# facebookresearch/brainmagick

Measured on AMD Instinct MI355X. Metric: segments/s, 208-ch x 360-sample SimpleConv + ClipLoss training step, higher is better.
Workload: dtype f32 (fp32-accurate: operands split into 2 scaled f16 planes, 3 MFMA products, fp32 accumulate; same parity tolerances as exact fp32, see DESIGN.md §2); 1 GPU; cfg2: gwilliams2022-shaped MEG C=208 T=360, F=120 features, 27 subjects, clip_conv SimpleConv (8985590 params) + ClipLoss + Adam; batch_per_gpu=256, global_batch=256, negatives=local, parallelism=dp1, comm=none, rccl_world=1, candidate_gather=none, distinct_batches=8

## Files before the change

### brainmagick_amd/csrc/bm_block.h

```cpp
#pragma once
#include "bm_common.h"

template <int V> struct BmVec;
template <> struct BmVec<1> {
    typedef float F;
    typedef unsigned char M;
};
template <> struct BmVec<4> {
    typedef f32x4 F;
    typedef uchar4 M;
};
__device__ __forceinline__ float bm_get(const float& v, int) { return v; }
__device__ __forceinline__ float bm_get(const f32x4& v, int i) { return v[i]; }
__device__ __forceinline__ unsigned char bm_get(const unsigned char& v, int) { return v; }
__device__ __forceinline__ unsigned char bm_get(const uchar4& v, int i) {
    return i == 0 ? v.x : i == 1 ? v.y : i == 2 ? v.z : v.w;
}
__device__ __forceinline__ void bm_set(float& v, int, float x) { v = x; }
__device__ __forceinline__ void bm_set(f32x4& v, int i, float x) { v[i] = x; }

template <int N, typename T, typename Op>
__device__ __forceinline__ T bm_pairwise(const T* v, Op op) {
    if constexpr (N == 1) return v[0];
    else return op(bm_pairwise<N / 2>(v, op), bm_pairwise<N - N / 2>(v + N / 2, op));
}
template <int WAVES, typename T, typename Op>
__device__ __forceinline__ T bm_block_fold(T wv, T* sh, Op op) {
    bm_wave_to_lds(wv, sh);
    __syncthreads();
    wv = bm_pairwise<WAVES>(sh, op);
    __syncthreads();
    return wv;
}
__device__ __forceinline__ float bm_max2(float a, float b) { return fmaxf(a, b); }
template <int WAVES>
__device__ __forceinline__ float bm_block_max(float v, float* sh) {
    return bm_block_fold<WAVES>(bm_wave_max(v), sh, bm_max2);
}
template <int WAVES>
__device__ __forceinline__ float bm_block_sum(float v, float* sh) {
    return bm_block_fold<WAVES>(bm_wave_sum(v), sh, [](float a, float b) { return a + b; });
}
template <int WAVES>
__device__ __forceinline__ double bm_block_sum(double v, double* sh) {
    return bm_block_fold<WAVES>(bm_wave_sum_d(v), sh, [](double a, double b) { return a + b; });
}

template <typename P>
struct BmFoldWs {
    unsigned* tickets;
    P* part;
    static constexpr long bytes(long n_partials) { return 64 + n_partials * (long)sizeof(P); }
    static BmFoldWs at(void* base) {
        return base ? BmFoldWs{(unsigned*)base, (P*)((char*)base + 64)} : BmFoldWs{nullptr, nullptr};
    }
};
template <typename T, int WAVES, int N = 1>
struct BmFoldLds {
    T wave[N][WAVES];
    int last;
};

template <typename P>
__device__ __forceinline__ void bm_store_partial(P* dst, P v) {
    __hip_atomic_store(dst, v, __ATOMIC_RELAXED, __HIP_MEMORY_SCOPE_AGENT);
}
__device__ __forceinline__ bool bm_last_arriver(unsigned* ticket, unsigned nblocks, int* sh_flag) {
    if (threadIdx.x == 0) {
        asm volatile("s_waitcnt vmcnt(0)" ::: "memory");
        const unsigned prev = __hip_atomic_fetch_add(ticket, 1u, __ATOMIC_RELAXED, __HIP_MEMORY_SCOPE_AGENT);
        const bool last = prev == nblocks - 1;
        if (last) {
            __builtin_amdgcn_fence(__ATOMIC_ACQUIRE, "agent");
            asm volatile("s_waitcnt vmcnt(0)" ::: "memory");
            __hip_atomic_store(ticket, 0u, __ATOMIC_RELAXED, __HIP_MEMORY_SCOPE_AGENT);
        }
        *sh_flag = last;
    }
    __syncthreads();
    return *sh_flag != 0;
}

template <int WAVES>
__device__ __forceinline__ bool bm_amax_arrive(float mx, float* part_dst, unsigned* ticket, unsigned nblocks,
                                               BmFoldLds<float, WAVES>& sh) {
    bm_wave_to_lds(bm_wave_max(mx), sh.wave[0]);
    __syncthreads();
    if (threadIdx.x == 0) bm_store_partial(part_dst, bm_pairwise<WAVES>(sh.wave[0], bm_max2));
    return bm_last_arriver(ticket, nblocks, &sh.last);
}
template <int WAVES>
__device__ __forceinline__ void bm_amax_slot_store(float m, float* out, float* sh) {
    bm_wave_to_lds(bm_wave_max(m), sh);
    __syncthreads();
    if (threadIdx.x < BM_AMAX_SHARDS) {
        float v = 0.f;
        if (threadIdx.x == 0) v = bm_pairwise<WAVES>(sh, bm_max2);
        out[threadIdx.x] = v;
    }
}
template <int WAVES>
__device__ __forceinline__ void bm_amax_fold(const float* part, int n, float* out, float* sh) {
    float m = 0.f;
    for (int i = threadIdx.x; i < n; i += WAVES * 64) m = fmaxf(m, part[i]);
    bm_amax_slot_store<WAVES>(m, out, sh);
}
template <int WAVES>
__device__ __forceinline__ void bm_amax_fold_rows(const float* part, int rows, int nsplit, int row_stride,
                                                  int split_stride, float* out, float* rows_out, float* sh) {
    float m = 0.f;
    for (int r = threadIdx.x; r < rows; r += WAVES * 64) {
        float v = 0.f;
        for (int k = 0; k < nsplit; ++k) v = fmaxf(v, part[r * row_stride + k * split_stride]);
        if (rows_out) rows_out[r] = v;
        m = fmaxf(m, v);
    }
    bm_amax_slot_store<WAVES>(m, out, sh);
}
```

### brainmagick_amd/csrc/conv_nn_h2w.hip

```cpp
#include "conv_h2_common.h"

#ifdef HG_TRACE
__device__ unsigned ch_trace_buf[64 * 4 * 24];
extern "C" int bm_debug_trace_read_conv(unsigned* out) {
    return (int)hipMemcpyFromSymbol(out, HIP_SYMBOL(ch_trace_buf), sizeof(unsigned) * 64 * 4 * 24);
}
#endif

__device__ __forceinline__ void ch_split_hi(float x0, float x1, float s, unsigned& hi) {
    asm("v_fma_mixlo_f16 %0, %1, %3, 0\n\t"
        "v_fma_mixhi_f16 %0, %2, %3, 0" : "=&v"(hi) : "v"(x0), "v"(x1), "v"(s));
}
__device__ __forceinline__ void ch_split_lo(float x0, float x1, float s, unsigned hi, unsigned& lo) {
    asm("v_fma_mixlo_f16 %0, %2, %4, -%1 op_sel_hi:[0,0,1]\n\t"
        "v_fma_mixhi_f16 %0, %3, %4, -%1 op_sel:[0,0,1] op_sel_hi:[0,0,1]"
        : "=&v"(lo) : "v"(hi), "v"(x0), "v"(x1), "v"(s));
}

enum { H2R_NONE = 0, H2R_WLOAD, H2R_SPLIT, H2R_WRITE, H2R_BAR, H2R_BREAD };
struct H2RItem { int kind, arg; };
template <int KS, int J, int NB>
constexpr int h2r_nitems() {
    if (KS == 1) return 32 + 4 + 1 + NB;
    return J == 0 ? 16 + NB : J == 1 ? 16 + 4 + 1 + NB : NB;
// ... 84 lines not shown
#define H2R_SOFF(C16_, J_) (((((C16_) >> 1) * KS + (J_)) * 8 + ((C16_) & 1) * 2) * a.Mpad * 16)
#define H2R_LOAD_X(R_, CB_) xreg[R_] = __builtin_bit_cast(float, __builtin_amdgcn_raw_buffer_load_b32(xr, (CB_) + (R_) * crow, 0, 0));
    const u32x4* xrd = Xs + h * HXWP + wn * (NW * 32) + nl;
    u32x4* xwr = Xs + tid;

    bm_static_for<16>([&](auto rc) __attribute__((always_inline)) { H2R_LOAD_X(decltype(rc)::value, xoff0) });
    bm_static_for<NA>([&](auto kc) __attribute__((always_inline)) { H2R_LOAD_A(0, decltype(kc)::value, 0) });
    bm_static_for<8>([&](auto uc) __attribute__((always_inline)) {
        constexpr int u = decltype(uc)::value;
        ch_split_hi(xreg[2 * u], xreg[2 * u + 1], sx, ph[u]);
        ch_split_lo(xreg[2 * u], xreg[2 * u + 1], sx, ph[u], pw[u]);
    });
    xwr[(0 * 2 + 0) * HXWP] = u32x4{ph[0], ph[1], ph[2], ph[3]};
    xwr[(1 * 2 + 0) * HXWP] = u32x4{pw[0], pw[1], pw[2], pw[3]};
    xwr[(0 * 2 + 1) * HXWP] = u32x4{ph[4], ph[5], ph[6], ph[7]};
    xwr[(1 * 2 + 1) * HXWP] = u32x4{pw[4], pw[5], pw[6], pw[7]};
    if (KS == 1) bm_static_for<16>([&](auto rc) __attribute__((always_inline)) { H2R_LOAD_X(decltype(rc)::value, 16 * crow + xoff0) });
    asm volatile("s_waitcnt lgkmcnt(0)\n\ts_barrier" ::: "memory");
    bm_static_for<NB>([&](auto ic) __attribute__((always_inline)) {
        constexpr int i = decltype(ic)::value;
        bf[0][i / NW][i % NW] = __builtin_bit_cast(f16x8, xrd[(i / NW) * 2 * HXWP + (i % NW) * 32]);
    });

#ifdef HG_TRACE
    unsigned tr[8], tacc[3][8];
    for (int i = 0; i < 3; ++i) for (int k = 0; k < 8; ++k) tacc[i][k] = 0;
    __builtin_amdgcn_sched_barrier(0);
    const unsigned t_loop0 = (unsigned)__builtin_readcyclecounter();
#endif
    auto stage = [&](int c16, auto jc, auto pc) __attribute__((always_inline)) {
        constexpr int j = decltype(jc)::value, par = decltype(pc)::value;
        CH_T(0)
        const bool last_chunk = c16 + 1 >= n16;
        const int nc16 = (j == KS - 1 && !last_chunk) ? c16 + 1 : c16;
        const int soff = (j == KS - 1) ? H2R_SOFF(nc16, last_chunk ? KS - 1 : 0) : H2R_SOFF(c16, j + 1);
        const u32x4* xnext = xrd + ((j == KS - 1 ? c16 + 1 : c16) & 1) * HXSLAB + (j == KS - 1 ? 0 : (j + 1) * a.dil);
        const int cb = (c16 + (KS == 1 ? 2 : 1)) * 16 * crow + xoff0;
        u32x4* xw = xwr + ((c16 + 1) & 1) * HXSLAB;
        bm_static_for<NS>([&](auto nc) __attribute__((always_inline)) {
            constexpr int n = decltype(nc)::value;
            constexpr int term = n / TN, w = n % TN, mt = w / NW, nt = w % NW;
            constexpr int pa = term == 0 ? 1 : 0, pb = term == 1 ? 1 : 0;
            acc[mt][nt] = __builtin_amdgcn_mfma_f32_32x32x16_f16(af[par][pa][mt], bf[par][pb][nt], acc[mt][nt], 0, 0, 0);
            if constexpr (n % 4 == 0) {
                if constexpr (n / 4 < NA) H2R_LOAD_A(par ^ 1, n / 4, soff)
            } else {
                constexpr int f = (n / 4) * 3 + n % 4 - 1;
                constexpr int L = h2r_nitems<KS, j, NB>();
                constexpr int i0 = (f * L + NF - 1) / NF, i1 = ((f + 1) * L + NF - 1) / NF;
                bm_static_for<i1 - i0>([&](auto ic) __attribute__((always_inline)) {
                    constexpr H2RItem it = h2r_item<KS, j, NB>(i0 + decltype(ic)::value);
                    if constexpr (it.kind == H2R_WLOAD) {
                        H2R_LOAD_X(it.arg, cb)
                    } else if constexpr (it.kind == H2R_SPLIT) {
                        constexpr int u = it.arg / 2;
                        if constexpr (it.arg % 2 == 0) ch_split_hi(xreg[2 * u], xreg[2 * u + 1], sx, ph[u]);
                        else ch_split_lo(xreg[2 * u], xreg[2 * u + 1], sx, ph[u], pw[u]);
                    } else if constexpr (it.kind == H2R_WRITE) {
                        constexpr int kg = it.arg / 2, plane = it.arg % 2;
                        if constexpr (plane == 0) xw[(0 * 2 + kg) * HXWP] = u32x4{ph[4 * kg], ph[4 * kg + 1], ph[4 * kg + 2], ph[4 * kg + 3]};
                        else xw[(1 * 2 + kg) * HXWP] = u32x4{pw[4 * kg], pw[4 * kg + 1], pw[4 * kg + 2], pw[4 * kg + 3]};
                    } else if constexpr (it.kind == H2R_BAR) {
                        asm volatile("s_waitcnt lgkmcnt(0)\n\ts_barrier" ::: "memory");
                    } else if constexpr (it.kind == H2R_BREAD) {
                        constexpr int p = it.arg / NW, q = it.arg % NW;
                        bf[par ^ 1][p][q] = __builtin_bit_cast(f16x8, xnext[p * 2 * HXWP + q * 32]);
                    }
                });
            }
            __builtin_amdgcn_sched_barrier(0);
        });
        CH_T(4)
#ifdef HG_TRACE
        tacc[j][0] += tr[4] - tr[0]; tacc[j][7] += 1;
#endif
    };
    auto chunk = [&](int c16, auto cpc) __attribute__((always_inline)) {
        constexpr int cp = decltype(cpc)::value;
        bm_static_for<KS>([&](auto jc) __attribute__((always_inline)) {
            constexpr int j = decltype(jc)::value;
            stage(c16, jc, std::integral_constant<int, (cp + j) & 1>{});
        });
    };
    for (int c16 = 0; c16 < n16; c16 += 2) {
        chunk(c16, std::integral_constant<int, 0>{});
        chunk(c16 + 1, std::integral_constant<int, KS & 1>{});
    }
#ifdef HG_TRACE
    __builtin_amdgcn_sched_barrier(0);
    const unsigned t_loop1 = (unsigned)__builtin_readcyclecounter();
    if (blockIdx.x < 64 && lane == 0)
        for (int i = 0; i < 3; ++i) for (int k = 0; k < 8; ++k) ch_trace_buf[((blockIdx.x * 4 + wave) * 3 + i) * 8 + k] = tacc[i][k];
#endif
    asm volatile("s_waitcnt vmcnt(0) lgkmcnt(0)\n\ts_barrier" ::: "memory");
#undef H2R_LOAD_A
#undef H2R_SOFF
#undef H2R_LOAD_X

#ifdef HG_TRACE
    h2_tile_epilogue<MW, RESK>(args, acc, smem, b, g, m0, n0, ntile, sx_inv, tid, lane, wm, wn, nl, h, ch_trace_buf);
#else
    h2_tile_epilogue<MW, RESK>(args, acc, smem, b, g, m0, n0, ntile, sx_inv, tid, lane, wm, wn, nl, h);
#endif
#ifdef HG_TRACE
    asm volatile("s_waitcnt vmcnt(0)" ::: "memory");
    if (blockIdx.x < 64 && lane == 0) {
        unsigned* o = ch_trace_buf + ((blockIdx.x * 4 + wave) * 3) * 8;
        o[5] = t_loop0 - t_kernel0;
        o[6] = (unsigned)__builtin_readcyclecounter() - t_loop1;
        o[8 + 5] = t_loop1 - t_loop0;
    }
#endif
}

extern "C" int bm_conv_h2_mw_for(int M) {
    int best = 5;
    long best_pad = -1;
    const int cand[3] = {5, 4, 2};
    for (int i = 0; i < 3; ++i) {
        const long bm = 64L * cand[i];
        const long pad = (long)cdiv(M, bm) * bm;
        if (best_pad < 0 || pad < best_pad) { best_pad = pad; best = cand[i]; }
    }
    return best;
}
extern "C" int bm_conv_h2_mpad(int M) {
    const int bm = 64 * bm_conv_h2_mw_for(M);
    return cdiv(M, bm) * bm;
}

extern "C" int bm_conv_h2_covers(int Cin, int M, int T, int KS, int dil) {
    if (KS != 1 && KS != 3) return 0;
    if ((KS >> 1) * dil > 16 || T <= 128) return 0;
    if ((long)Cin * T * 4 >= 0x40000000L) return 0;
    if ((long)Cin * KS > 3840) return 0;
    return (long)bm_conv_h2_mpad(M) * 2 <= (long)M * 3 || M >= 96;
}

extern "C" int bm_conv_h2_stats_tiles(int B, int T) { return B * cdiv(T, HBN) * 2; }

extern "C" long bm_packed_weight_bytes_h2(int G, int M, int Cin, int KS) {
    const long mpad = bm_conv_h2_mpad(M);
    return (long)G * cdiv(Cin, 32) * KS * 2 * 4 * mpad * 8 * 2 + (long)G * mpad * 4;
}

struct PackH2Job {
    const float* src;
    unsigned short* dst;
    float* wscale;
    const float* alpha;
    long sg, sm, sc, sj;
    int M, Cin, KS, flip, Mpad, nchunk;
    int block0, nblocks;
};

#define PACK_ROWS 4
#define PACK_MAX_NK 3840

__device__ __forceinline__ void pack_h2_rows(const PackH2Job& jb, int block, float* tile, float* rs) {
    const float* __restrict__ src = jb.src;
    const int M = jb.M, Cin = jb.Cin, KS = jb.KS, Mpad = jb.Mpad, nchunk = jb.nchunk, flip = jb.flip;
    const long sg = jb.sg, sm = jb.sm, sc = jb.sc, sj = jb.sj;
    const int rows_per_group = Mpad / PACK_ROWS;
    const int g = block / rows_per_group, m0 = (block - g * rows_per_group) * PACK_ROWS;
    const float alpha = jb.alpha ? *jb.alpha : 1.f;
    const int nk = Cin * KS;
    const int tid = threadIdx.x, lane = tid & 63, wave = tid >> 6;
    const float* base = src + g * sg + (long)m0 * sm;
    const bool rows_inside = sm < sc;
    for (int idx = tid; idx < PACK_ROWS * nk; idx += blockDim.x) {
        int r, c, j;
        if (rows_inside) {
            j = idx % KS;
            const int t = idx / KS;
            r = t % PACK_ROWS;
            c = t / PACK_ROWS;
        } else {
            j = idx % KS;
            const int t = idx / KS;
            c = t % Cin;
            r = t / Cin;
        }
        tile[r * nk + c * KS + j] = (m0 + r < M) ? alpha * base[r * sm + c * sc + j * sj] : 0.f;
    }
    __syncthreads();
    {
        float mx = 0.f;
        for (int i = lane; i < nk; i += 64) mx = fmaxf(mx, fabsf(tile[wave * nk + i]));
        mx = bm_wave_max(mx);
        float s, inv;
        bm_scale_from_amax(mx, s, inv);
        if (lane == 0) {
            rs[wave] = s;
            jb.wscale[(long)g * Mpad + m0 + wave] = inv;
        }
    }
    __syncthreads();
    const int nslots = nchunk * KS * 4;
    const long plane_stride = (long)4 * Mpad * 8;
    for (int t = tid; t < PACK_ROWS * nslots; t += blockDim.x) {
        const int r = t % PACK_ROWS, q = t / PACK_ROWS;
        const int kg = q & 3;
        const int j = (q >> 2) % KS;
        const int chunk = (q >> 2) / KS;
        const int jj = flip ? KS - 1 - j : j;
        const float sr = rs[r];
        alignas(16) unsigned short hi[8];
        alignas(16) unsigned short lo[8];
#pragma unroll
        for (int e8 = 0; e8 < 8; ++e8) {
            const int c = chunk * 32 + kg * 8 + e8;
            const float v = c < Cin ? tile[r * nk + c * KS + jj] * sr : 0.f;
            const _Float16 a = (_Float16)v;
            const _Float16 l = (_Float16)(v - (float)a);
            hi[e8] = __builtin_bit_cast(unsigned short, a);
            lo[e8] = __builtin_bit_cast(unsigned short, l);
        }
        const long stage = ((long)g * nchunk + chunk) * KS + j;
        unsigned short* out = jb.dst + stage * 2 * plane_stride + ((long)kg * Mpad + m0 + r) * 8;
        *reinterpret_cast<uint4*>(out) = *reinterpret_cast<const uint4*>(hi);
        *reinterpret_cast<uint4*>(out + plane_stride) = *reinterpret_cast<const uint4*>(lo);
    }
}

__global__ __launch_bounds__(256) void pack_weights_h2_kernel(PackH2Job jb) {
    extern __shared__ float pack_smem[];
    pack_h2_rows(jb, blockIdx.x, pack_smem + PACK_ROWS, pack_smem);
}

__global__ __launch_bounds__(256) void pack_weights_h2_batch_kernel(const PackH2Job* __restrict__ jobs, int njobs) {
    extern __shared__ float pack_smem[];
    int lo = 0, hi = njobs - 1;
    while (lo < hi) {
        const int mid = (lo + hi + 1) >> 1;
        if (jobs[mid].block0 <= (int)blockIdx.x) lo = mid; else hi = mid - 1;
    }
    const PackH2Job jb = jobs[lo];
    pack_h2_rows(jb, blockIdx.x - jb.block0, pack_smem + PACK_ROWS, pack_smem);
}

static int pack_h2_fill(PackH2Job& jb, const float* src, void* dst, int G, int M, int Cin, int KS, long sg, long sm,
                        long sc, long sj, int flip, const float* alpha_ptr) {
    BM_REQUIRE(src && dst, "pack_weights_h2: null pointer");
    BM_REQUIRE(G > 0 && M > 0 && Cin > 0 && KS > 0, "pack_weights_h2: bad dims");
    jb.Mpad = bm_conv_h2_mpad(M);
    jb.nchunk = cdiv(Cin, 32);
    const long f16_elems = (long)G * jb.nchunk * KS * 2 * 4 * jb.Mpad * 8;
    jb.src = src; jb.dst = (unsigned short*)dst;
    jb.wscale = reinterpret_cast<float*>(reinterpret_cast<char*>(dst) + f16_elems * 2);
    jb.alpha = alpha_ptr;
    jb.sg = sg; jb.sm = sm; jb.sc = sc; jb.sj = sj;
    jb.M = M; jb.Cin = Cin; jb.KS = KS; jb.flip = flip;
    BM_REQUIRE(Cin * KS <= PACK_MAX_NK, "pack_weights_h2: Cin * KS = %d exceeds %d", Cin * KS, PACK_MAX_NK);
    jb.block0 = 0; jb.nblocks = G * jb.Mpad / PACK_ROWS;
    return BM_OK;
}

extern "C" int bm_pack_weights_h2(const float* src, void* dst, int G, int M, int Cin, int KS, long sg, long sm,
                                  long sc, long sj, int flip, const float* alpha_ptr, void* stream) {
    PackH2Job jb;
    if (int rc = pack_h2_fill(jb, src, dst, G, M, Cin, KS, sg, sm, sc, sj, flip, alpha_ptr)) return rc;
    hipLaunchKernelGGL(pack_weights_h2_kernel, dim3((unsigned)jb.nblocks), dim3(256),
                       (size_t)(PACK_ROWS + PACK_ROWS * Cin * KS) * sizeof(float), (hipStream_t)stream, jb);
    return bm_check_launch("pack_weights_h2");
}

extern "C" int bm_pack_h2_job_bytes() { return (int)sizeof(PackH2Job); }

extern "C" int bm_pack_h2_job_fill(void* job, const float* src, void* dst, int G, int M, int Cin, int KS, long sg,
                                   long sm, long sc, long sj, int flip, const float* alpha_ptr, int block0) {
    if (!job) return -1;
    PackH2Job jb;
    if (pack_h2_fill(jb, src, dst, G, M, Cin, KS, sg, sm, sc, sj, flip, alpha_ptr)) return -1;
    jb.block0 = block0;
    memcpy(job, &jb, sizeof(jb));
    return jb.nblocks;
}

extern "C" int bm_pack_weights_h2_batch(const void* jobs_dev, int njobs, int total_blocks, int max_nk, void* stream) {
    BM_REQUIRE(jobs_dev && njobs > 0 && total_blocks > 0, "pack_weights_h2_batch: bad arguments");
    BM_REQUIRE(max_nk > 0 && max_nk <= PACK_MAX_NK, "pack_weights_h2_batch: max_nk = %d (largest Cin * KS of the jobs)", max_nk);
    hipLaunchKernelGGL(pack_weights_h2_batch_kernel, dim3((unsigned)total_blocks), dim3(256),
                       (size_t)(PACK_ROWS + PACK_ROWS * max_nk) * sizeof(float), (hipStream_t)stream,
                       (const PackH2Job*)jobs_dev, njobs);
    return bm_check_launch("pack_weights_h2_batch");
}

__global__ __launch_bounds__(1024) void amax_kernel(const float* __restrict__ x, long n, float* __restrict__ ws,
                                                    int* __restrict__ nonfinite) {
    __shared__ float sh[16];
    float mx = 0.f;
    unsigned top = 0u;
    long head = (long)((16u - (unsigned)((uintptr_t)x & 15u)) & 15u) >> 2;
    if (head > n) head = n;
    const long n4 = (n - head) >> 2;
    const float4* x4 = reinterpret_cast<const float4*>(x + head);
    for (long i = (long)blockIdx.x * blockDim.x + threadIdx.x; i < n4; i += (long)gridDim.x * blockDim.x) {
        const float4 v = x4[i];
        mx = fmaxf(fmaxf(mx, fabsf(v.x)), fmaxf(fabsf(v.y), fmaxf(fabsf(v.z), fabsf(v.w))));
        top = max(max(top, __float_as_uint(v.x) & 0x7fffffffu),
                  max(__float_as_uint(v.y) & 0x7fffffffu, max(__float_as_uint(v.z) & 0x7fffffffu,
                                                               __float_as_uint(v.w) & 0x7fffffffu)));
    }
    if (blockIdx.x == 0) {
        const long tail0 = head + (n4 << 2);
        for (long i = threadIdx.x; i < head + (n - tail0); i += blockDim.x) {
            const long k = i < head ? i : tail0 + (i - head);
            mx = fmaxf(mx, fabsf(x[k]));
            top = max(top, __float_as_uint(x[k]) & 0x7fffffffu);
        }
    }
    if (nonfinite && top >= 0x7f800000u) atomicOr(nonfinite, 1);
    bm_publish_amax(mx, ws, sh);
}

extern "C" int bm_amax_checked(const float* x, long n, float* out, float* ws, int* nonfinite_flag, void* stream) {
    BM_REQUIRE(x && out && ws && n >= 0, "amax: bad arguments");
    BM_REQUIRE(((uintptr_t)x & 3) == 0, "amax: x must be 4-byte aligned");
    hipStream_t s = (hipStream_t)stream;
    long blocks = (n / 4 + 1023) / 1024;
    blocks = blocks < 1 ? 1 : (blocks > 256 ? 256 : blocks);
    hipLaunchKernelGGL(amax_kernel, dim3((unsigned)blocks), dim3(1024), 0, s, x, n, ws, nonfinite_flag);
    if (int rc = bm_check_launch("amax")) return rc;
    return bm_amax_finalize(ws, (int)blocks, out, s);
}

extern "C" int bm_amax(const float* x, long n, float* out, float* ws, void* stream) {
    return bm_amax_checked(x, n, out, ws, nullptr, stream);
}

template <int KS, int MW>
static int launch_conv_nn_h2w(ConvH2Args args, float* y_amax_out, hipStream_t stream) {
    constexpr int HBM = 64 * MW;
    size_t lds = (size_t)(3 * 2 * 2 * HBM + 2 * HXSLAB) * 16;
    const size_t lds_ep = (size_t)(4 * HBM + 4) * sizeof(float);
    if (lds < lds_ep) lds = lds_ep;
    static const bool ldsdma = [] { const char* e = getenv("BM_CONV_LDSDMA"); return e && e[0] == '1'; }();
    if (!ldsdma) lds = (size_t)(2 * HXSLAB) * 16 > lds_ep ? (size_t)(2 * HXSLAB) * 16 : lds_ep;
    const ConvNNArgs& c = args.c;
    const bool resk = KS == 3 && !ldsdma && c.res && c.y_out && !c.y_pre && !c.ep_scale && !c.stats && c.act == BM_ACT_NONE;
    static bool attr_set = false;
    if (!ldsdma && !attr_set) {
        hipError_t e = hipFuncSetAttribute(reinterpret_cast<const void*>(conv_nn_h2w_kernel<KS, MW, false>),
                                           hipFuncAttributeMaxDynamicSharedMemorySize, (int)lds);
        if (e == hipSuccess && KS == 3)
            e = hipFuncSetAttribute(reinterpret_cast<const void*>(conv_nn_h2w_kernel<KS, MW, KS == 3>),
                                    hipFuncAttributeMaxDynamicSharedMemorySize, (int)lds);
        if (e != hipSuccess) return bm_set_error((int)e, "conv_nn_h2w: hipFuncSetAttribute: %s", hipGetErrorString(e));
        attr_set = true;
    }
    args.c.ntiles_n = cdiv(args.c.T, HBN);
    args.c.ntiles_m = args.c.Mpad / HBM;
    const long nblocks = (long)args.c.B * args.c.ntiles_n * args.c.ntiles_m;
    if (nblocks <= 0) return BM_OK;
    const bool publish = y_amax_out && args.y_amax.ws && nblocks <= BM_AMAX_WS;
    float* ws = args.y_amax.ws;
    if (!publish) args.y_amax = BmAmaxDst{nullptr};
    if (ldsdma) {
        if (int rc = bm_launch_conv_nn_h2d(args, KS, MW, lds, (unsigned)nblocks, stream)) return rc;
    } else if (resk)
        hipLaunchKernelGGL((conv_nn_h2w_kernel<KS, MW, KS == 3>), dim3((unsigned)nblocks), dim3(256), lds, stream, args);
    else
        hipLaunchKernelGGL((conv_nn_h2w_kernel<KS, MW, false>), dim3((unsigned)nblocks), dim3(256), lds, stream, args);
    if (int rc = bm_check_launch("conv_nn_h2w")) return rc;
    if (publish) return bm_amax_done(args.y_amax, (int)nblocks, y_amax_out, stream);
    if (y_amax_out && ws)
        return bm_amax(args.c.y_out, (long)args.c.B * args.c.M * args.c.T, y_amax_out, ws, stream);
    return BM_OK;
}

extern "C" int bm_conv1d_nn_h2(const float* x, long x_bstride, const float* x_amax, const void* wpacked,
                               const int* widx, const float* bias, long bias_gstride, const float* ep_scale, const float* ep_shift,
                               const float* res, long res_bstride, float* y_pre, float* y_out, long y_bstride,
                               float* stats, int B, int Cin, int M, int T, int KS, int dil, int act, float leak,
                               int G, float* y_amax_out, float* amax_ws, void* stream) {
    BM_REQUIRE(x && wpacked && x_amax, "conv1d_nn_h2: null x / w / x_amax");
    BM_REQUIRE(y_pre || y_out, "conv1d_nn_h2: no output");
    BM_REQUIRE(!stats || (y_pre && !y_out && !ep_scale && act == BM_ACT_NONE && !res),
               "conv1d_nn_h2: per-tile statistics come with y_pre alone (the training-mode BatchNorm layers)");
    BM_REQUIRE(B >= 0 && Cin > 0 && M > 0 && T > 0 && dil >= 1 && G >= 1, "conv1d_nn_h2: bad dims");
    BM_REQUIRE((ep_scale == nullptr) == (ep_shift == nullptr), "conv1d_nn_h2: scale/shift must come together");
    BM_REQUIRE(bm_conv_h2_covers(Cin, M, T, KS, dil), "conv1d_nn_h2: shape not covered (Cin=%d M=%d T=%d KS=%d dil=%d)",
               Cin, M, T, KS, dil);
    ConvH2Args args;
    ConvNNArgs& a = args.c;
    a.x = x; a.x_bstride = x_bstride; a.wp = (const float*)wpacked; a.widx = widx; a.bias = bias; a.bias_gstride = bias_gstride;
    a.ep_scale = ep_scale; a.ep_shift = ep_shift; a.res = res; a.res_bstride = res_bstride;
    a.y_pre = y_pre; a.y_out = y_out; a.y_bstride = y_bstride; a.stats = stats;
    a.B = B; a.Cin = Cin; a.M = M; a.T = T; a.KS = KS; a.dil = dil; a.act = act; a.leak = leak;
    const int mw = bm_conv_h2_mw_for(M);
    a.Mpad = bm_conv_h2_mpad(M);
    a.nchunk = cdiv(Cin, 32);
    const long f16_elems = (long)G * a.nchunk * KS * 2 * 4 * a.Mpad * 8;
    args.x_amax = x_amax;
    BM_REQUIRE(!y_amax_out || amax_ws, "conv1d_nn_h2: y_amax_out needs the amax workspace");
    if (!y_out) y_amax_out = nullptr;
    args.y_amax = bm_amax_dst(y_amax_out, amax_ws);
    args.wscale = reinterpret_cast<const float*>(reinterpret_cast<const char*>(wpacked) + f16_elems * 2);
    hipStream_t s = (hipStream_t)stream;
#define H2_DISPATCH(MW_)                                                                 \
    return KS == 1 ? launch_conv_nn_h2w<1, MW_>(args, y_amax_out, s) : launch_conv_nn_h2w<3, MW_>(args, y_amax_out, s);
    switch (mw) {
        case 5: H2_DISPATCH(5)
        case 4: H2_DISPATCH(4)
        default: H2_DISPATCH(2)
    }
#undef H2_DISPATCH
}
```

### brainmagick_amd/csrc/core.hip

```cpp
#include "bm_block.h"
#include <stdarg.h>
#include <stdlib.h>

thread_local char bm_err_buf[512] = {0};

int bm_set_error(int code, const char* fmt, ...) {
    va_list ap;
    va_start(ap, fmt);
    vsnprintf(bm_err_buf, sizeof(bm_err_buf), fmt, ap);
    va_end(ap);
    return code;
}

int bm_check_launch(const char* what) {
    hipError_t e = hipGetLastError();
    if (e != hipSuccess) return bm_set_error((int)e, "%s: launch failed: %s", what, hipGetErrorString(e));
    return BM_OK;
}

extern "C" const char* bm_last_error(void) { return bm_err_buf; }
extern "C" int bm_version(void) { return 111; }

extern "C" int bm_device_count(void) {
    int n = 0;
    hipError_t e = hipGetDeviceCount(&n);
    if (e != hipSuccess) { bm_set_error((int)e, "hipGetDeviceCount: %s", hipGetErrorString(e)); return -1; }
    return n;
}

#define FIN_THREADS 1024
#define FIN_WAVES (FIN_THREADS / 64)
__global__ __launch_bounds__(FIN_THREADS) void amax_finalize_kernel(const float* __restrict__ ws, int n,
                                                                    float* __restrict__ out) {
    __shared__ float sh[FIN_WAVES];
    bm_amax_fold<FIN_WAVES>(ws, n, out, sh);
}

int bm_amax_finalize(const float* ws, int n, float* out, hipStream_t stream) {
    if (!out) return BM_OK;
    hipLaunchKernelGGL(amax_finalize_kernel, dim3(1), dim3(FIN_THREADS), 0, stream, ws, n, out);
    return bm_check_launch("amax_finalize");
}

__global__ __launch_bounds__(FIN_THREADS) void amax_finalize_rows_kernel(const float* __restrict__ ws, int C, int nsplit,
                                                                         float* __restrict__ out,
                                                                         float* __restrict__ rows_out,
                                                                         const double* __restrict__ sum_partial,
                                                                         float* __restrict__ sums_out) {
    __shared__ float sh[FIN_WAVES];
    if (sum_partial)
        for (int c = threadIdx.x; c < C; c += FIN_THREADS) {
            double t = 0;
            for (int s = 0; s < nsplit; ++s) t += sum_partial[(long)c * nsplit + s];
            sums_out[c] = (float)t;
        }
    bm_amax_fold_rows<FIN_WAVES>(ws, C, nsplit, 1, C, out, rows_out, sh);
}

int bm_amax_finalize_rows(const float* ws, int C, int nsplit, float* out, float* rows_out, hipStream_t stream) {
    if (!out) return BM_OK;
    hipLaunchKernelGGL(amax_finalize_rows_kernel, dim3(1), dim3(FIN_THREADS), 0, stream, ws, C, nsplit, out, rows_out,
                       (const double*)nullptr, (float*)nullptr);
    return bm_check_launch("amax_finalize_rows");
}

int bm_amax_finalize_rows_sums(const float* ws, int C, int nsplit, float* out, float* rows_out,
                               const double* sum_partial, float* sums_out, hipStream_t stream) {
    hipLaunchKernelGGL(amax_finalize_rows_kernel, dim3(1), dim3(FIN_THREADS), 0, stream, ws, C, nsplit, out, rows_out,
                       sum_partial, sums_out);
    return bm_check_launch("amax_finalize_rows");
}

extern "C" int bm_amax_ws_elems(void) { return BM_AMAX_WS; }
```

### brainmagick_amd/csrc/norm_act.hip

```cpp
#include <cstdlib>
#include "bm_common.h"

template <int VEC> struct Pack;
template <> struct Pack<1> {
    float v[1];
    __device__ static Pack ld(const float* p) { Pack r; r.v[0] = *p; return r; }
    __device__ void st(float* p) const { *p = v[0]; }
};
template <> struct Pack<4> {
    float v[4];
    __device__ static Pack ld(const float* p) {
        const float4 t = *reinterpret_cast<const float4*>(p);
        Pack r; r.v[0] = t.x; r.v[1] = t.y; r.v[2] = t.z; r.v[3] = t.w; return r;
    }
    __device__ void st(float* p) const { *reinterpret_cast<float4*>(p) = make_float4(v[0], v[1], v[2], v[3]); }
};

#define LAUNCH_VEC(vec4, kernel, grid, stream, ...)                                              \
    do {                                                                                         \
        if (vec4) hipLaunchKernelGGL(kernel<4>, grid, dim3(256), 0, stream, __VA_ARGS__);        \
        else hipLaunchKernelGGL(kernel<1>, grid, dim3(256), 0, stream, __VA_ARGS__);             \
    } while (0)
static int flat_blocks(long n) { return (int)((n + 255) / 256 > 16384 ? 16384 : (n + 255) / 256); }

struct SlabWalk {
    int bl, tv, dbl, dtv, TV;
    __device__ SlabWalk(int TV_, int first, int step) : TV(TV_) {
        bl = first / TV_; tv = first - bl * TV_;
        dbl = step / TV_; dtv = step - dbl * TV_;
    }
    __device__ void next() {
        tv += dtv; bl += dbl;
        if (tv >= TV) { tv -= TV; ++bl; }
    }
};

struct Slab {
    int b0, nb, TV;
    __device__ Slab(int B, int split, int nsplit, int T, int VEC)
        : b0((int)((long)B * split / nsplit)), nb((int)((long)B * (split + 1) / nsplit) - b0), TV(T / VEC) {}
};

#ifndef BWD_UNROLL
#define BWD_UNROLL 4
#endif

#define SLAB_TRIPS_BEGIN2(sl, AT, AT2, Data, LOAD)                              \
    SlabWalk w((sl).TV, threadIdx.x, blockDim.x);                               \
    while (w.bl < (sl).nb) {                                                    \
        long off[BWD_UNROLL];                                                   \
        bool ok[BWD_UNROLL];                                                    \
        long off2[BWD_UNROLL];                                                  \
        Data data[BWD_UNROLL];                                                  \
        _Pragma("unroll") for (int q = 0; q < BWD_UNROLL; ++q) {                \
            ok[q] = w.bl < (sl).nb;                                             \
            off[q] = ok[q] ? AT(w.bl, w.tv) : off[0];                           \
            off2[q] = ok[q] ? AT2(w.bl, w.tv) : off2[0];                        \
            LOAD(data[q], off[q], off2[q]);                                     \
            if (ok[q]) w.next();                                                \
        }                                                                       \
        _Pragma("unroll") for (int q = 0; q < BWD_UNROLL; ++q) {                \
            if (!ok[q]) continue;
#define SLAB_NO_OFF2(bl, tv) 0L
#define SLAB_TRIPS_BEGIN(sl, AT, Data, LOAD) SLAB_TRIPS_BEGIN2(sl, AT, SLAB_NO_OFF2, Data, LOAD)
#define SLAB_TRIPS_END \
        }              \
    }

template <int NV>
__device__ void block_sum(double (&v)[NV], double* sh) {
    const int lane = threadIdx.x & 63, wave = threadIdx.x >> 6, nw = blockDim.x >> 6;
#pragma unroll
    for (int i = 0; i < NV; ++i) v[i] = bm_wave_sum_d(v[i]);
    __syncthreads();
    if (lane == 0)
#pragma unroll
        for (int i = 0; i < NV; ++i) sh[wave * NV + i] = v[i];
    __syncthreads();
    if (threadIdx.x == 0) {
#pragma unroll
        for (int i = 0; i < NV; ++i) {
            double s = 0;
            for (int w = 0; w < nw; ++w) s += sh[w * NV + i];
            v[i] = s;
        }
    }
}

__global__ void bn_finalize_kernel(const float* __restrict__ stats, long tstride, long cstride, int ntiles, int C, double count,
                                   const float* __restrict__ gamma, const float* __restrict__ beta,
                                   float* running_mean, float* running_var, long* num_batches,
                                   float momentum, float eps, float* __restrict__ mean_out,
                                   float* __restrict__ invstd_out, float* __restrict__ scale_out,
                                   float* __restrict__ shift_out) {
    const int c = blockIdx.x;
    double s = 0, s2 = 0;
    for (int t = threadIdx.x; t < ntiles; t += blockDim.x) {
        s += (double)stats[(long)t * tstride + (long)c * cstride + 0];
        s2 += (double)stats[(long)t * tstride + (long)c * cstride + 1];
    }
    s = bm_wave_sum_d(s);
    s2 = bm_wave_sum_d(s2);
    if (threadIdx.x == 0) {
        const double mean = s / count;
        double var = s2 / count - mean * mean;
        if (var < 0) var = 0;
        const float invstd = (float)(1.0 / sqrt(var + (double)eps));
        const float g = gamma ? gamma[c] : 1.f, bt = beta ? beta[c] : 0.f;
        const float sc = g * invstd;
        mean_out[c] = (float)mean;
        invstd_out[c] = invstd;
        scale_out[c] = sc;
        shift_out[c] = bt - (float)mean * sc;
        if (running_mean && isfinite(mean) && isfinite(var)) {
            const double unbiased = count > 1 ? var * count / (count - 1) : var;
            running_mean[c] = (1.f - momentum) * running_mean[c] + momentum * (float)mean;
            running_var[c] = (1.f - momentum) * running_var[c] + momentum * (float)unbiased;
        }
        if (num_batches && c == 0) *num_batches += 1;
    }
}

static int bn_finalize(const char* what, const float* stats, long tstride, long cstride, int ntiles, int C, long count,
                       const float* gamma, const float* beta, float* running_mean, float* running_var,
                       long* num_batches, float momentum, float eps, float* mean, float* invstd, float* scale,
                       float* shift, void* stream) {
    BM_REQUIRE(stats && mean && invstd && scale && shift, "%s: null pointer", what);
    BM_REQUIRE(C > 0 && ntiles > 0 && count > 0, "%s: bad dims", what);
    hipLaunchKernelGGL(bn_finalize_kernel, dim3(C), dim3(64), 0, (hipStream_t)stream, stats, tstride, cstride, ntiles, C,
                       (double)count, gamma, beta, running_mean, running_var, num_batches, momentum,
                       eps, mean, invstd, scale, shift);
    return bm_check_launch(what);
}

extern "C" int bm_bn_finalize(const float* stats, int ntiles, int C, long count, const float* gamma,
                              const float* beta, float* running_mean, float* running_var,
                              long* num_batches, float momentum, float eps, float* mean,
                              float* invstd, float* scale, float* shift, void* stream) {
    return bn_finalize("bn_finalize", stats, (long)C * 2, 2L, ntiles, C, count, gamma, beta, running_mean, running_var,
                       num_batches, momentum, eps, mean, invstd, scale, shift, stream);
}

extern "C" int bm_bn_finalize_cm(const float* stats, int ntiles, int C, long count, const float* gamma,
                                 const float* beta, float* running_mean, float* running_var,
                                 long* num_batches, float momentum, float eps, float* mean,
                                 float* invstd, float* scale, float* shift, void* stream) {
    return bn_finalize("bn_finalize_cm", stats, 2L, (long)ntiles * 2, ntiles, C, count, gamma, beta, running_mean,
                       running_var, num_batches, momentum, eps, mean, invstd, scale, shift, stream);
}

__global__ void bn_eval_affine_kernel(int C, const float* gamma, const float* beta,
                                      const float* running_mean, const float* running_var,
                                      float eps, float* mean, float* invstd, float* scale,
                                      float* shift) {
    const int c = blockIdx.x * blockDim.x + threadIdx.x;
    if (c >= C) return;
    const float is = 1.0f / sqrtf(running_var[c] + eps);
    const float sc = (gamma ? gamma[c] : 1.f) * is;
    mean[c] = running_mean[c];
    invstd[c] = is;
    scale[c] = sc;
    shift[c] = (beta ? beta[c] : 0.f) - running_mean[c] * sc;
}

extern "C" int bm_bn_eval_affine(int C, const float* gamma, const float* beta,
                                 const float* running_mean, const float* running_var, float eps,
                                 float* mean, float* invstd, float* scale, float* shift,
                                 void* stream) {
    BM_REQUIRE(running_mean && running_var && scale && shift, "bn_eval_affine: null pointer");
    hipLaunchKernelGGL(bn_eval_affine_kernel, dim3(cdiv(C, 256)), dim3(256), 0, (hipStream_t)stream, C,
                       gamma, beta, running_mean, running_var, eps, mean, invstd, scale, shift);
    return bm_check_launch("bn_eval_affine");
}

template <int VEC>
__global__ void affine_act_res_kernel(const float* __restrict__ y, const float* __restrict__ scale,
                                      const float* __restrict__ shift, const float* __restrict__ res,
                                      float* __restrict__ out, long nvec, int C, int T, int act,
                                      float leak, BmAmaxDst amax_ws, BmFastDiv div_tv, BmFastDiv div_c) {
    __shared__ float amax_sh[4];
    float amx = 0.f;
    for (long e = (long)blockIdx.x * blockDim.x + threadIdx.x; e < nvec;
         e += (long)gridDim.x * blockDim.x) {
        const unsigned row = bm_div((unsigned)e, div_tv);
        const int c = (int)(row - bm_div(row, div_c) * (unsigned)C);
        const float sc = scale ? scale[c] : 1.f, sh = scale ? shift[c] : 0.f;
        Pack<VEC> v = Pack<VEC>::ld(y + e * VEC);
        Pack<VEC> r;
        if (res) r = Pack<VEC>::ld(res + e * VEC);
#pragma unroll
        for (int i = 0; i < VEC; ++i) {
            float z = bm_act(v.v[i] * sc + sh, act, leak);
            if (res) z += r.v[i];
            v.v[i] = z;
            amx = fmaxf(amx, fabsf(z));
        }
        v.st(out + e * VEC);
    }
    bm_publish_amax(amx, amax_ws, amax_sh);
}

extern "C" int bm_affine_act_res(const float* y, const float* scale, const float* shift,
                                 const float* res, float* out, int B, int C, int T, int act,
                                 float leak, float* amax_out, float* amax_ws, void* stream) {
    BM_REQUIRE(y && out, "affine_act_res: null pointer");
    BM_REQUIRE(!amax_out || amax_ws, "affine_act_res: amax_out needs the amax workspace");
    const long n = (long)B * C * T;
    if (n == 0) return BM_OK;
    BM_REQUIRE(n < 0xffffffffL, "affine_act_res: tensor of %ld elements (32-bit element index)", n);
    hipStream_t s = (hipStream_t)stream;
    const BmAmaxDst amax_dst = bm_amax_dst(amax_out, amax_ws);
    const int vec = T % 4 == 0 ? 4 : 1;
    const long nvec = n / vec;
    const int nblk = flat_blocks(nvec);
    LAUNCH_VEC(vec == 4, affine_act_res_kernel, dim3(nblk), s, y, scale, shift, res, out, nvec, C, T, act, leak, amax_dst,
               bm_fastdiv((unsigned)(T / vec)), bm_fastdiv((unsigned)C));
    if (int rc = bm_check_launch("affine_act_res")) return rc;
    return bm_amax_done(amax_dst, nblk, amax_out, s);
}

#define NSPLIT_MAX 32

template <int VEC> struct BnPos { Pack<VEC> d, v; };
#define BN_POS_AT(bl, tv) (((long)(sl.b0 + (bl)) * C + c) * T + (long)(tv) * VEC)
#define BN_POS_LOAD(p, off, unused) p.d = Pack<VEC>::ld(dout + off); p.v = Pack<VEC>::ld(y + off)

template <int VEC>
__global__ __launch_bounds__(256) void bn_bwd_reduce_kernel(
    const float* __restrict__ dout, const float* __restrict__ y, const float* __restrict__ scale,
    const float* __restrict__ shift, const float* __restrict__ mean, const float* __restrict__ invstd,
    double* __restrict__ partial, int B, int C, int T, int act, float leak) {
    __shared__ double sh[4 * 2];
    const int c = blockIdx.x, split = blockIdx.y, nsplit = gridDim.y;
    const Slab sl(B, split, nsplit, T, VEC);
    const float sc = scale ? scale[c] : 1.f, shf = scale ? shift[c] : 0.f;
    const float mu = mean ? mean[c] : 0.f, is = invstd ? invstd[c] : 1.f;
    float s0 = 0.f, s1 = 0.f;
    SLAB_TRIPS_BEGIN(sl, BN_POS_AT, BnPos<VEC>, BN_POS_LOAD)
        const BnPos<VEC>& p = data[q];
#pragma unroll
        for (int i = 0; i < VEC; ++i) {
            const float dz = p.d.v[i] * bm_act_grad(p.v.v[i] * sc + shf, act, leak);
            s0 += dz;
            s1 += dz * ((p.v.v[i] - mu) * is);
        }
    SLAB_TRIPS_END
    double acc[2] = {s0, s1};
    block_sum<2>(acc, sh);
    if (threadIdx.x == 0) {
        partial[((long)c * nsplit + split) * 2 + 0] = acc[0];
        partial[((long)c * nsplit + split) * 2 + 1] = acc[1];
    }
// ... 524 lines not shown
```

Measured before the change: 17010 segments/s.

## Batch loads in flight across fold, finalize, and weight-pack kernels

Several small reduction and packing kernels are changed to issue multiple independent loads before consuming them: the amax fold uses 16-byte vector loads, the per-row fold spreads each row's splits across lanes with a shuffle reduction, and the BN and sums finalizers batch float2/double loads. The batched weight-pack kernel now handles 4, 8 or 16 rows per block, uses fast division and a padded LDS stride, and keeps eight loads in flight per thread. The goal is to hide global memory latency in these latency-bound tail kernels, at the cost of more registers, more LDS, and more complex indexing.

```diff
diff --git a/brainmagick_amd/csrc/bm_block.h b/brainmagick_amd/csrc/bm_block.h
--- a/brainmagick_amd/csrc/bm_block.h
+++ b/brainmagick_amd/csrc/bm_block.h
@@ -99,20 +99,54 @@
         out[threadIdx.x] = v;
     }
 }
+#define BM_FOLD_INFLIGHT 4
+#define BM_FOLD_ROWS_INFLIGHT 8
 template <int WAVES>
 __device__ __forceinline__ void bm_amax_fold(const float* part, int n, float* out, float* sh) {
+    constexpr int NT = WAVES * 64;
     float m = 0.f;
-    for (int i = threadIdx.x; i < n; i += WAVES * 64) m = fmaxf(m, part[i]);
+    const int n4 = ((uintptr_t)part & 15) == 0 ? n >> 2 : 0;
+    const f32x4* p4 = reinterpret_cast<const f32x4*>(part);
+    for (int base = 0; base < n4; base += NT * BM_FOLD_INFLIGHT) {
+        f32x4 v[BM_FOLD_INFLIGHT];
+#pragma unroll
+        for (int q = 0; q < BM_FOLD_INFLIGHT; ++q) {
+            const int i = base + q * NT + (int)threadIdx.x;
+            v[q] = p4[i < n4 ? i : base];
+        }
+#pragma unroll
+        for (int q = 0; q < BM_FOLD_INFLIGHT; ++q)
+            m = fmaxf(fmaxf(m, fmaxf(v[q][0], v[q][1])), fmaxf(v[q][2], v[q][3]));
+    }
+    for (int i = n4 * 4 + threadIdx.x; i < n; i += NT) m = fmaxf(m, part[i]);
     bm_amax_slot_store<WAVES>(m, out, sh);
 }
 template <int WAVES>
 __device__ __forceinline__ void bm_amax_fold_rows(const float* part, int rows, int nsplit, int row_stride,
                                                   int split_stride, float* out, float* rows_out, float* sh) {
+    constexpr int NT = WAVES * 64;
+    int L = 1;
+    while (L < 64 && L < nsplit && (long)rows * (L * 2) <= NT) L *= 2;
+    const int j = threadIdx.x & (L - 1), r0 = threadIdx.x / L, rstep = NT / L;
     float m = 0.f;
-    for (int r = threadIdx.x; r < rows; r += WAVES * 64) {
+    for (int rb = 0; rb < rows; rb += rstep) {
+        const int r = rb + r0;
+        const bool inside = r < rows && j < nsplit;
+        const float* row = part + (inside ? r * row_stride : 0);
         float v = 0.f;
-        for (int k = 0; k < nsplit; ++k) v = fmaxf(v, part[r * row_stride + k * split_stride]);
-        if (rows_out) rows_out[r] = v;
+        for (int k0 = inside ? j : 0; k0 < nsplit; k0 += L * BM_FOLD_ROWS_INFLIGHT) {
+            float t[BM_FOLD_ROWS_INFLIGHT];
+#pragma unroll
+            for (int q = 0; q < BM_FOLD_ROWS_INFLIGHT; ++q) {
+                const int k = k0 + q * L;
+                t[q] = row[(k < nsplit ? k : k0) * split_stride];
+            }
+#pragma unroll
+            for (int q = 0; q < BM_FOLD_ROWS_INFLIGHT; ++q) v = fmaxf(v, t[q]);
+        }
+        if (!inside) v = 0.f;
+        for (int o = L >> 1; o > 0; o >>= 1) v = fmaxf(v, __shfl_xor(v, o));
+        if (rows_out && inside && j == 0) rows_out[r] = v;
         m = fmaxf(m, v);
     }
     bm_amax_slot_store<WAVES>(m, out, sh);
diff --git a/brainmagick_amd/csrc/conv_nn_h2w.hip b/brainmagick_amd/csrc/conv_nn_h2w.hip
--- a/brainmagick_amd/csrc/conv_nn_h2w.hip
+++ b/brainmagick_amd/csrc/conv_nn_h2w.hip
@@ -260,57 +260,85 @@
     long sg, sm, sc, sj;
     int M, Cin, KS, flip, Mpad, nchunk;
     int block0, nblocks;
+    int rows;
+    BmFastDiv dks, dcin;
 };
 
-#define PACK_ROWS 4
+#define PACK_MAX_ROWS 16
 #define PACK_MAX_NK 3840
-
+#define PACK_WIDE_FLOATS (2 * PACK_MAX_NK)
+#define PACK_INFLIGHT 8
+static inline int pack_rows_for(int nk) {
+    return 16 * nk <= PACK_WIDE_FLOATS ? 16 : (8 * nk <= PACK_WIDE_FLOATS ? 8 : 4);
+}
+static inline size_t pack_lds_bytes(int max_nk) {
+    const long cap = PACK_WIDE_FLOATS;
+    const long wide = 16L * max_nk < cap ? 16L * max_nk : cap;
+    const long fl = wide > 4L * max_nk ? wide : 4L * max_nk;
+    return (size_t)(2 * PACK_MAX_ROWS + fl) * sizeof(float);
+}
+
+template <int ROWS>
 __device__ __forceinline__ void pack_h2_rows(const PackH2Job& jb, int block, float* tile, float* rs) {
     const float* __restrict__ src = jb.src;
     const int M = jb.M, Cin = jb.Cin, KS = jb.KS, Mpad = jb.Mpad, nchunk = jb.nchunk, flip = jb.flip;
     const long sg = jb.sg, sm = jb.sm, sc = jb.sc, sj = jb.sj;
-    const int rows_per_group = Mpad / PACK_ROWS;
-    const int g = block / rows_per_group, m0 = (block - g * rows_per_group) * PACK_ROWS;
+    const BmFastDiv dks = jb.dks, dcin = jb.dcin;
+    const int rows_per_group = Mpad / ROWS;
+    const int g = block / rows_per_group, m0 = (block - g * rows_per_group) * ROWS;
     const float alpha = jb.alpha ? *jb.alpha : 1.f;
     const int nk = Cin * KS;
+    const int ld = nk | 1;
     const int tid = threadIdx.x, lane = tid & 63, wave = tid >> 6;
-    const float* base = src + g * sg + (long)m0 * sm;
+    const float* gbase = src + g * sg;
     const bool rows_inside = sm < sc;
-    for (int idx = tid; idx < PACK_ROWS * nk; idx += blockDim.x) {
-        int r, c, j;
-        if (rows_inside) {
-            j = idx % KS;
-            const int t = idx / KS;
-            r = t % PACK_ROWS;
-            c = t / PACK_ROWS;
-        } else {
-            j = idx % KS;
-            const int t = idx / KS;
-            c = t % Cin;
-            r = t / Cin;
+    const int total = ROWS * nk;
+    for (int idx0 = tid; idx0 < total; idx0 += PACK_INFLIGHT * 256) {
+        float v[PACK_INFLIGHT];
+        int at[PACK_INFLIGHT];
+#pragma unroll
+        for (int q = 0; q < PACK_INFLIGHT; ++q) {
+            const int idx = idx0 + q * 256;
+            const unsigned t = bm_div((unsigned)idx, dks);
+            const int j = idx - (int)t * KS;
+            int r, c;
+            if (rows_inside) {
+                r = (int)(t % ROWS);
+                c = (int)(t / ROWS);
+            } else {
+                r = (int)bm_div(t, dcin);
+                c = (int)t - r * Cin;
+            }
+            const bool ok = idx < total && m0 + r < M;
+            at[q] = idx < total ? r * ld + c * KS + j : -1;
+            v[q] = gbase[ok ? (long)(m0 + r) * sm + c * sc + j * sj : 0L];
+            if (!ok) v[q] = 0.f;
+            else v[q] = alpha * v[q];
         }
-        tile[r * nk + c * KS + j] = (m0 + r < M) ? alpha * base[r * sm + c * sc + j * sj] : 0.f;
+#pragma unroll
+        for (int q = 0; q < PACK_INFLIGHT; ++q)
+            if (at[q] >= 0) tile[at[q]] = v[q];
     }
     __syncthreads();
-    {
+    for (int r = wave; r < ROWS; r += 4) {
         float mx = 0.f;
-        for (int i = lane; i < nk; i += 64) mx = fmaxf(mx, fabsf(tile[wave * nk + i]));
+        for (int i = lane; i < nk; i += 64) mx = fmaxf(mx, fabsf(tile[r * ld + i]));
         mx = bm_wave_max(mx);
         float s, inv;
         bm_scale_from_amax(mx, s, inv);
         if (lane == 0) {
-            rs[wave] = s;
-            jb.wscale[(long)g * Mpad + m0 + wave] = inv;
+            rs[r] = s;
+            jb.wscale[(long)g * Mpad + m0 + r] = inv;
         }
     }
     __syncthreads();
     const int nslots = nchunk * KS * 4;
     const long plane_stride = (long)4 * Mpad * 8;
-    for (int t = tid; t < PACK_ROWS * nslots; t += blockDim.x) {
-        const int r = t % PACK_ROWS, q = t / PACK_ROWS;
+    for (int t = tid; t < ROWS * nslots; t += 256) {
+        const int r = t % ROWS, q = t / ROWS;
         const int kg = q & 3;
-        const int j = (q >> 2) % KS;
-        const int chunk = (q >> 2) / KS;
+        const int chunk = (int)bm_div((unsigned)(q >> 2), dks);
+        const int j = (q >> 2) - chunk * KS;
         const int jj = flip ? KS - 1 - j : j;
         const float sr = rs[r];
         alignas(16) unsigned short hi[8];
@@ -318,7 +346,7 @@
 #pragma unroll
         for (int e8 = 0; e8 < 8; ++e8) {
             const int c = chunk * 32 + kg * 8 + e8;
-            const float v = c < Cin ? tile[r * nk + c * KS + jj] * sr : 0.f;
+            const float v = c < Cin ? tile[r * ld + c * KS + jj] * sr : 0.f;
             const _Float16 a = (_Float16)v;
             const _Float16 l = (_Float16)(v - (float)a);
             hi[e8] = __builtin_bit_cast(unsigned short, a);
@@ -330,10 +358,15 @@
         *reinterpret_cast<uint4*>(out + plane_stride) = *reinterpret_cast<const uint4*>(lo);
     }
 }
+__device__ __forceinline__ void pack_h2_job(const PackH2Job& jb, int block, float* smem) {
+    if (jb.rows == 16) pack_h2_rows<16>(jb, block, smem + PACK_MAX_ROWS, smem);
+    else if (jb.rows == 8) pack_h2_rows<8>(jb, block, smem + PACK_MAX_ROWS, smem);
+    else pack_h2_rows<4>(jb, block, smem + PACK_MAX_ROWS, smem);
+}
 
 __global__ __launch_bounds__(256) void pack_weights_h2_kernel(PackH2Job jb) {
     extern __shared__ float pack_smem[];
-    pack_h2_rows(jb, blockIdx.x, pack_smem + PACK_ROWS, pack_smem);
+    pack_h2_rows<4>(jb, blockIdx.x, pack_smem + PACK_MAX_ROWS, pack_smem);
 }
 
 __global__ __launch_bounds__(256) void pack_weights_h2_batch_kernel(const PackH2Job* __restrict__ jobs, int njobs) {
@@ -344,11 +377,11 @@
         if (jobs[mid].block0 <= (int)blockIdx.x) lo = mid; else hi = mid - 1;
     }
     const PackH2Job jb = jobs[lo];
-    pack_h2_rows(jb, blockIdx.x - jb.block0, pack_smem + PACK_ROWS, pack_smem);
+    pack_h2_job(jb, blockIdx.x - jb.block0, pack_smem);
 }
 
 static int pack_h2_fill(PackH2Job& jb, const float* src, void* dst, int G, int M, int Cin, int KS, long sg, long sm,
-                        long sc, long sj, int flip, const float* alpha_ptr) {
+                        long sc, long sj, int flip, const float* alpha_ptr, bool batched) {
     BM_REQUIRE(src && dst, "pack_weights_h2: null pointer");
     BM_REQUIRE(G > 0 && M > 0 && Cin > 0 && KS > 0, "pack_weights_h2: bad dims");
     jb.Mpad = bm_conv_h2_mpad(M);
@@ -360,16 +393,18 @@
     jb.sg = sg; jb.sm = sm; jb.sc = sc; jb.sj = sj;
     jb.M = M; jb.Cin = Cin; jb.KS = KS; jb.flip = flip;
     BM_REQUIRE(Cin * KS <= PACK_MAX_NK, "pack_weights_h2: Cin * KS = %d exceeds %d", Cin * KS, PACK_MAX_NK);
-    jb.block0 = 0; jb.nblocks = G * jb.Mpad / PACK_ROWS;
+    jb.rows = batched ? pack_rows_for(Cin * KS) : 4;
+    jb.dks = bm_fastdiv((unsigned)KS); jb.dcin = bm_fastdiv((unsigned)Cin);
+    jb.block0 = 0; jb.nblocks = G * jb.Mpad / jb.rows;
     return BM_OK;
 }
 
 extern "C" int bm_pack_weights_h2(const float* src, void* dst, int G, int M, int Cin, int KS, long sg, long sm,
                                   long sc, long sj, int flip, const float* alpha_ptr, void* stream) {
     PackH2Job jb;
-    if (int rc = pack_h2_fill(jb, src, dst, G, M, Cin, KS, sg, sm, sc, sj, flip, alpha_ptr)) return rc;
+    if (int rc = pack_h2_fill(jb, src, dst, G, M, Cin, KS, sg, sm, sc, sj, flip, alpha_ptr, false)) return rc;
     hipLaunchKernelGGL(pack_weights_h2_kernel, dim3((unsigned)jb.nblocks), dim3(256),
-                       (size_t)(PACK_ROWS + PACK_ROWS * Cin * KS) * sizeof(float), (hipStream_t)stream, jb);
+                       (size_t)(2 * PACK_MAX_ROWS + 4L * Cin * KS) * sizeof(float), (hipStream_t)stream, jb);
     return bm_check_launch("pack_weights_h2");
 }
 
@@ -379,7 +414,7 @@
                                    long sm, long sc, long sj, int flip, const float* alpha_ptr, int block0) {
     if (!job) return -1;
     PackH2Job jb;
-    if (pack_h2_fill(jb, src, dst, G, M, Cin, KS, sg, sm, sc, sj, flip, alpha_ptr)) return -1;
+    if (pack_h2_fill(jb, src, dst, G, M, Cin, KS, sg, sm, sc, sj, flip, alpha_ptr, true)) return -1;
     jb.block0 = block0;
     memcpy(job, &jb, sizeof(jb));
     return jb.nblocks;
@@ -389,7 +424,7 @@
     BM_REQUIRE(jobs_dev && njobs > 0 && total_blocks > 0, "pack_weights_h2_batch: bad arguments");
     BM_REQUIRE(max_nk > 0 && max_nk <= PACK_MAX_NK, "pack_weights_h2_batch: max_nk = %d (largest Cin * KS of the jobs)", max_nk);
     hipLaunchKernelGGL(pack_weights_h2_batch_kernel, dim3((unsigned)total_blocks), dim3(256),
-                       (size_t)(PACK_ROWS + PACK_ROWS * max_nk) * sizeof(float), (hipStream_t)stream,
+                       pack_lds_bytes(max_nk), (hipStream_t)stream,
                        (const PackH2Job*)jobs_dev, njobs);
     return bm_check_launch("pack_weights_h2_batch");
 }
diff --git a/brainmagick_amd/csrc/core.hip b/brainmagick_amd/csrc/core.hip
--- a/brainmagick_amd/csrc/core.hip
+++ b/brainmagick_amd/csrc/core.hip
@@ -30,6 +30,7 @@
 
 #define FIN_THREADS 1024
 #define FIN_WAVES (FIN_THREADS / 64)
+#define FIN_SUMS_INFLIGHT 16
 __global__ __launch_bounds__(FIN_THREADS) void amax_finalize_kernel(const float* __restrict__ ws, int n,
                                                                     float* __restrict__ out) {
     __shared__ float sh[FIN_WAVES];
@@ -50,8 +51,16 @@
     __shared__ float sh[FIN_WAVES];
     if (sum_partial)
         for (int c = threadIdx.x; c < C; c += FIN_THREADS) {
+            const double* row = sum_partial + (long)c * nsplit;
             double t = 0;
-            for (int s = 0; s < nsplit; ++s) t += sum_partial[(long)c * nsplit + s];
+            for (int s0 = 0; s0 < nsplit; s0 += FIN_SUMS_INFLIGHT) {
+                double v[FIN_SUMS_INFLIGHT];
+#pragma unroll
+                for (int q = 0; q < FIN_SUMS_INFLIGHT; ++q) v[q] = row[s0 + q < nsplit ? s0 + q : s0];
+#pragma unroll
+                for (int q = 0; q < FIN_SUMS_INFLIGHT; ++q)
+                    if (s0 + q < nsplit) t += v[q];
+            }
             sums_out[c] = (float)t;
         }
     bm_amax_fold_rows<FIN_WAVES>(ws, C, nsplit, 1, C, out, rows_out, sh);
diff --git a/brainmagick_amd/csrc/norm_act.hip b/brainmagick_amd/csrc/norm_act.hip
--- a/brainmagick_amd/csrc/norm_act.hip
+++ b/brainmagick_amd/csrc/norm_act.hip
@@ -87,6 +87,7 @@
     }
 }
 
+#define BN_FIN_INFLIGHT 16
 __global__ void bn_finalize_kernel(const float* __restrict__ stats, long tstride, long cstride, int ntiles, int C, double count,
                                    const float* __restrict__ gamma, const float* __restrict__ beta,
                                    float* running_mean, float* running_var, long* num_batches,
@@ -95,9 +96,23 @@
                                    float* __restrict__ shift_out) {
     const int c = blockIdx.x;
     double s = 0, s2 = 0;
-    for (int t = threadIdx.x; t < ntiles; t += blockDim.x) {
-        s += (double)stats[(long)t * tstride + (long)c * cstride + 0];
-        s2 += (double)stats[(long)t * tstride + (long)c * cstride + 1];
+    const float* chan = stats + (long)c * cstride;
+    const bool pair8 = (((uintptr_t)stats & 7) | ((tstride | cstride) & 1)) == 0;
+    for (int t0 = threadIdx.x; t0 < ntiles; t0 += BN_FIN_INFLIGHT * (int)blockDim.x) {
+        float2 v[BN_FIN_INFLIGHT];
+#pragma unroll
+        for (int q = 0; q < BN_FIN_INFLIGHT; ++q) {
+            const int t = t0 + q * (int)blockDim.x;
+            const float* p = chan + (long)(t < ntiles ? t : t0) * tstride;
+            if (pair8) v[q] = *reinterpret_cast<const float2*>(p);
+            else v[q] = make_float2(p[0], p[1]);
+        }
+#pragma unroll
+        for (int q = 0; q < BN_FIN_INFLIGHT; ++q)
+            if (t0 + q * (int)blockDim.x < ntiles) {
+                s += (double)v[q].x;
+                s2 += (double)v[q].y;
+            }
     }
     s = bm_wave_sum_d(s);
     s2 = bm_wave_sum_d(s2);
```

Measured after the change: 16580 segments/s. 2.5% lower.
